# MartinMikkelsen/TensorTrainNumerics.jl

Measured on AMD Instinct MI355X. Metric: TT cores/sec for QTT Laplacian apply+round, d=30 rank-64, higher is better.
Workload: dtype f64

## Files before the change

### include/ttn.h

```cpp
#ifndef TTN_H
#define TTN_H

#include <stdint.h>

#ifdef __cplusplus
extern "C" {
#endif

#define TTN_OK                 0
#define TTN_ERR_DIMS          -1
#define TTN_ERR_BOND_INDEX    -2
#define TTN_ERR_SWEEPS        -3
#define TTN_ERR_CENTER        -4
#define TTN_ERR_CAPACITY      -5
#define TTN_ERR_ARG           -6
#define TTN_ERR_NOT_INIT      -7
#define TTN_ERR_UNSUPPORTED   -8
#define TTN_ERR_NO_CONVERGENCE -9
#define TTN_ERR_SINGULAR      -10

int         ttn_init(int device);
int         ttn_finalize(void);
const char* ttn_version(void);
const char* ttn_last_error_string(void);
// ... 126 lines not shown
int ttn_add(ttn_tt_t x, ttn_tt_t y, ttn_tt_t z);
int ttn_scale(double a, ttn_tt_t x, ttn_tt_t y);
int ttn_scale_batch(const double* a, ttn_tt_t x, ttn_tt_t y);
int ttn_orthogonalize(ttn_tt_t x, int64_t center, ttn_tt_t y);

int ttn_sv_capture(ttn_tt_t h, int enable);
int ttn_sv_get(ttn_tt_t h, int64_t b, int64_t step, double* out, int64_t cap, int64_t* n);

int ttn_timer_begin(void);
int ttn_timer_end(float* ms);
int ttn_event_record(int64_t slot);
int ttn_event_elapsed(int64_t slot_a, int64_t slot_b, float* ms);

int ttn_selftest_gemm(int64_t m, int64_t n, int64_t k, const double* A, const double* B, double* C, double alpha, double beta,
                      int ta, int tb);

int ttn_selftest_lu_solve(int64_t N, const double* K, const double* rhs, double* x_out, int64_t* piv_out, int form);
int ttn_selftest_two_site_apply(int64_t na, int64_t nb, int64_t Rz, const double* G, const double* H, const double* v, double* out);

int ttn_selftest_eig128(const double* G, int64_t n, int64_t r, int64_t nev, double* sig, double* X, int64_t* ticks_rc);
int ttn_selftest_sym_eig(int64_t N, int64_t k, const double* A, double* lam, double* Y);
int ttn_debug_ortho_state(int64_t b, int64_t* out4);

int ttn_apply_f64(int64_t d, const int64_t* dims,
                  const double* const* A_cores, const int64_t* A_rks,
                  const double* const* X_cores, const int64_t* X_rks,
                  double* const* Y_cores);
int ttn_dot_f64(int64_t d, const int64_t* dims,
                const double* const* A_cores, const int64_t* A_rks,
                const double* const* B_cores, const int64_t* B_rks, double* out);
// ... 65 lines not shown
```

### tensortrainnumerics.jl_amd/_lib.py

```python
from __future__ import annotations

import ctypes as C
import os
import subprocess

_HERE = os.path.dirname(os.path.abspath(__file__))
LIB_PATH = os.environ.get("TTN_LIB") or os.path.join(_HERE, "libttn_hip.so")
CSRC = os.path.join(_HERE, "csrc")
INCLUDE = os.path.join(os.path.dirname(_HERE), "include")

TTN_OK = 0
TTN_ERR_DIMS = -1
TTN_ERR_BOND_INDEX = -2
TTN_ERR_SWEEPS = -3
TTN_ERR_CENTER = -4
TTN_ERR_CAPACITY = -5
TTN_ERR_ARG = -6
TTN_ERR_NOT_INIT = -7
TTN_ERR_UNSUPPORTED = -8
TTN_ERR_NO_CONVERGENCE = -9
TTN_ERR_SINGULAR = -10

i64 = C.c_int64
p_i64 = C.POINTER(C.c_int64)
# ... 88 lines not shown
                                   C.c_void_p, C.c_void_p, C.c_void_p]),
    "ttn_cross_eval": (C.c_int, [C.c_int, i64, i64, pp_f64, p_i64, p_i64, C.c_void_p, C.c_void_p, C.c_void_p, C.c_void_p, C.c_double,
                                 C.c_void_p]),
    "ttn_tdvp_contract_f64": (C.c_int, [C.c_int, C.c_int, i64, p_i64, C.c_void_p, C.c_void_p, C.c_void_p, C.c_void_p, C.c_void_p, C.c_void_p, C.c_int]),
    "ttn_selftest_eig128": (C.c_int, [C.c_void_p, i64, i64, i64, C.c_void_p, C.c_void_p, C.c_void_p]),
    "ttn_selftest_sym_eig": (C.c_int, [i64, i64, C.c_void_p, C.c_void_p, C.c_void_p]),
    "ttn_add": (C.c_int, [handle, handle, handle]),
    "ttn_scale": (C.c_int, [C.c_double, handle, handle]),
    "ttn_scale_batch": (C.c_int, [p_f64, handle, handle]),
    "ttn_orthogonalize": (C.c_int, [handle, i64, handle]),
    "ttn_sv_capture": (C.c_int, [handle, C.c_int]),
    "ttn_sv_get": (C.c_int, [handle, i64, i64, p_f64, i64, p_i64]),
    "ttn_timer_begin": (C.c_int, []),
    "ttn_timer_end": (C.c_int, [C.POINTER(C.c_float)]),
    "ttn_selftest_gemm": (C.c_int, [i64, i64, i64, p_f64, p_f64, p_f64, C.c_double, C.c_double, C.c_int, C.c_int]),
    "ttn_selftest_lu_solve": (C.c_int, [i64, p_f64, p_f64, p_f64, p_i64, C.c_int]),
    "ttn_selftest_two_site_apply": (C.c_int, [i64, i64, i64, p_f64, p_f64, p_f64, p_f64]),
    "ttn_event_record": (C.c_int, [i64]),
    "ttn_event_elapsed": (C.c_int, [i64, i64, C.POINTER(C.c_float)]),
    "ttn_apply_f64": (C.c_int, [i64, p_i64, pp_f64, p_i64, pp_f64, p_i64, pp_f64]),
    "ttn_dot_f64": (C.c_int, [i64, p_i64, pp_f64, p_i64, pp_f64, p_i64, p_f64]),
    "ttn_hadamard_f64": (C.c_int, [i64, p_i64, pp_f64, p_i64, pp_f64, p_i64, pp_f64]),
    "ttn_add_f64": (C.c_int, [i64, p_i64, pp_f64, p_i64, pp_f64, p_i64, pp_f64]),
    "ttn_scale_f64": (C.c_int, [i64, p_i64, C.c_double, pp_f64, p_i64, p_i64, pp_f64, p_i64]),
    "ttn_orthogonalize_f64": (C.c_int, [i64, p_i64, pp_f64, p_i64, i64, pp_f64, p_i64, p_i64]),
    "ttn_compress_f64": (C.c_int, [i64, p_i64, pp_f64, p_i64, i64, C.c_double, i64]),
    "ttn_apply_compress_rank_bound": (C.c_int, [i64, p_i64, p_i64, p_i64, i64, i64, p_i64]),
    "ttn_apply_compress_f64": (C.c_int, [i64, p_i64, pp_f64, p_i64, pp_f64, p_i64, pp_f64, p_i64, i64, C.c_double, i64]),
    "ttn_bond_truncate_f64": (C.c_int, [i64, p_i64, pp_f64, p_i64, i64, i64, C.c_double]),
    "ttn_r_and_d_to_rks": (C.c_int, [i64, p_i64, i64, p_i64, i64, p_i64]),
# ... 131 lines not shown
```

### tensortrainnumerics.jl_amd/csrc/ttn_api.hip

```cpp
#include "../../include/ttn.h"
#include "ttn_common.h"
#include "ttn_stream_kernels.h"
#include "ttn_dense_kernels.h"
#include "ttn_swap_kernels.h"
#include "ttn_selftest_kernels.h"
#include "ttn_dot_kernels.h"
#include "ttn_ortho_kernels.h"
#include "ttn_ortho512.h"
#include "ttn_ortho_ramp.h"
#include "ttn_hsvd_kernels.h"
#include "ttn_resite_kernels.h"
#include "ttn_als_kernels.h"
#include "ttn_als_grid.h"
#include "ttn_eigsolve_kernels.h"
#include "ttn_als_eig_kernels.h"
#include "ttn_eig_kernels.h"
#include "ttn_tdvp_kernels.h"
#include "ttn_densefact_kernels.h"
#include "ttn_cross_kernels.h"
#include "ttn_cross_batch_kernels.h"
#include "ttn_opalg_kernels.h"
#include "ttn_cplx_kernels.h"
#include "ttn_grid_kernels.h"
#include "ttn_grad_kernels.h"
// ... 6 lines not shown
#include <cmath>
#include <cstdio>
#include <cstring>
#include <cstdlib>
#include <mutex>
#include <set>
#include <string>
#include <vector>

extern "C" {
int ttn_wg512_init(void);
size_t ttn_wg512_compress_args_bytes(void);
int ttn_wg512_launch_compress(const void* args, size_t nbytes, int grid, hipStream_t stream);
int ttn_wg512_selftest_eig(const double* G, double* Vst, int n, int r, int nev, double* sig, double* Xout, long long* clk, hipStream_t stream);
int ttn_wg512_selftest_gemm(int m, int n, int k, double* A, double* B, double* C, double alpha, double beta, int ta, int tb, hipStream_t stream);
}

namespace {
std::set<struct ttn_tt_s*> g_live;
std::recursive_mutex g_mu;
bool g_init = false;
int g_device = -1;
hipStream_t g_stream = nullptr;
hipEvent_t g_ev0 = nullptr, g_ev1 = nullptr;
hipEvent_t g_launch_ev0 = nullptr, g_launch_ev1 = nullptr;
bool g_have_launch_ms = false;
size_t g_ortho_state_off = 0;
int g_ortho_state_batch = 0;
long long g_dense_plan[3] = {-1, 0, 0};
long long g_gather_plan[4] = {0, 0, 0, 0};
// ... 174 lines not shown
        {(const void*)k_compress, COMPRESS_LDS_BYTES},
        {(const void*)k_selftest_eig128, COMPRESS_LDS_BYTES},
        {(const void*)k_mals_linsolve, COMPRESS_LDS_BYTES},
        {(const void*)k_als_linsolve, COMPRESS_LDS_BYTES},
        {(const void*)k_two_site_eig, COMPRESS_LDS_BYTES},
        {(const void*)k_als_eig, COMPRESS_LDS_BYTES},
        {(const void*)k_increase_ranks, COMPRESS_LDS_BYTES},
        {(const void*)k_ttv_decomp, COMPRESS_LDS_BYTES},
        {(const void*)k_split_sites, COMPRESS_LDS_BYTES},
        {(const void*)k_swap_chain, COMPRESS_LDS_BYTES},
        {(const void*)k_orthogonalize, ORTHO_LDS_BYTES},
        {(const void*)k_ortho512, O5_LDS_BYTES(TTN_MAX_D * 8)},
        {(const void*)k_dot_fused, DOT_LDS_BYTES(DOT_MAX_D)},
        {(const void*)k_grad_chain, DOT_LDS_BYTES(DOT_MAX_D)},
        {(const void*)k_selftest_gemm, sizeof(double) * GEMM_LDS_TOTAL},
        {(const void*)k_tdvp, TDVP_LDS_BYTES},
        {(const void*)k_lu_panel, LU_PANEL_LDS_BYTES},
        {(const void*)k_lu_trail, sizeof(double) * GEMM_LDS_TOTAL},
        {(const void*)k_selftest_lu, COMPRESS_LDS_BYTES},
        {(const void*)k_selftest_two_site_apply, COMPRESS_LDS_BYTES},
        {(const void*)k_cross_maxvol<false>, TTN_XV_LDS_BYTES},
        {(const void*)k_cross_maxvol<true>, TTN_XV_LDS_BYTES},
        {(const void*)k_zcompress, TTN_ZC_LDS_BYTES},
        {(const void*)k_cross_batch_site, TTN_XB_LDS_BYTES},
        {(const void*)k_expect<0>, EXPECT_LDS_BYTES(EXPECT_MAX_D)},
        {(const void*)k_expect<1>, EXPECT_LDS_BYTES(EXPECT_MAX_D)},
        {(const void*)k_expect<2>, EXPECT_LDS_BYTES(EXPECT_MAX_D)},
        {(const void*)k_expect<3>, EXPECT_LDS_BYTES(EXPECT_MAX_D)},
        {(const void*)k_expect<4>, EXPECT_LDS_BYTES(EXPECT_MAX_D)},
        {(const void*)k_expect<5>, EXPECT_LDS_BYTES(EXPECT_MAX_D)},
// ... 2565 lines not shown
    HIPCHK(hipMalloc((void**)&dC, sizeof(double) * m * n));
    HIPCHK(hipMemcpyAsync(dA, A, sizeof(double) * m * k, hipMemcpyHostToDevice, g_stream));
    HIPCHK(hipMemcpyAsync(dB, B, sizeof(double) * k * n, hipMemcpyHostToDevice, g_stream));
    HIPCHK(hipMemcpyAsync(dC, C, sizeof(double) * m * n, hipMemcpyHostToDevice, g_stream));
    if (getenv("TTN_WG512_SELFTEST") && atoi(getenv("TTN_WG512_SELFTEST"))) {
        const int rc512 = ttn_wg512_selftest_gemm((int)m, (int)n, (int)k, dA, dB, dC, alpha, beta, ta, tb, g_stream);
        if (rc512) return hipfail((hipError_t)rc512, "k_selftest_gemm (512-thread build)");
    } else {
    hipLaunchKernelGGL(k_selftest_gemm, dim3(1), dim3(TTN_WG), sizeof(double) * GEMM_LDS_TOTAL, g_stream, (int)m, (int)n, (int)k,
                       dA, dB, dC, alpha, beta, ta, tb);
    HIPCHK(hipGetLastError());
    }
    HIPCHK(hipMemcpyAsync(C, dC, sizeof(double) * m * n, hipMemcpyDeviceToHost, g_stream));
    HIPCHK(hipStreamSynchronize(g_stream));
    hipFree(dA); hipFree(dB); hipFree(dC);
    return TTN_OK;
}

int ttn_selftest_lu_solve(int64_t N, const double* K, const double* rhs, double* x_out, int64_t* piv_out, int form) {
    std::lock_guard<std::recursive_mutex> lk(g_mu);
    if (!K || !rhs || !x_out || !piv_out || N < 1 || (form != 0 && form != 1) || N > (form == 0 ? TTN_DENSE_LOCAL_MAX_ALS : 8192))
        return fail(TTN_ERR_ARG, "ttn_selftest_lu_solve: need 1 <= N <= 2048 (form 0) / 8192 (form 1) and form 0 or 1");
    NEED_INIT();
    { const int rc = g_lu_flag.ensure(sizeof(int)); if (rc) return rc; }
    int* d_flag = g_lu_flag.as<int>();
    double *dK = nullptr, *dR = nullptr;
    int* dP = nullptr;
    HIPCHK(hipMalloc((void**)&dK, sizeof(double) * N * N));
    HIPCHK(hipMalloc((void**)&dR, sizeof(double) * N));
    HIPCHK(hipMalloc((void**)&dP, sizeof(int) * N));
// ... 1311 lines not shown
```

### tensortrainnumerics.jl_amd/csrc/ttn_dense_kernels.h

```cpp
#pragma once
#include "ttn_wg_prims.h"
#include "ttn_wg_gemm.h"
#include "ttn_wg_lq.h"
#include "ttn_wg_jacobi.h"
#include "ttn_wg_chol.h"

struct CompressArgs {
    TTDev tt;
    long long max_bond;
    double truncerr;
    int sweeps;
    int k_single;
    int k_first, k_last;
    double* scratch;
    long long scratch_stride;
    int pmax, qmax;
    double* sv_out;
    int sv_steps;
    int* status;
    int* sweep_stats;
    int fast;
    int fused;
    TTODev op;
    TTDev x;
// ... 131 lines not shown

__device__ __noinline__ double wg_check_diag_tab(const double* sigs, const double* D, int ldd, int r, double s0, double* tab, double* red) {
    sigs = unip(sigs); D = unip(D); ldd = uni32(ldd); r = uni32(r); s0 = unif64(s0); tab = unip(tab); red = unip(red);
    lds_f64* t = (lds_f64*)tab; lds_f64* ref = t + 128;
    const int tid = threadIdx.x, lane = tid & 63, wave = tid >> 6;
    for (int i = tid; i < r; i += TTN_WG) { const double si = sigs[i]; t[i] = 1.0 / sqrt(s0 * si); ref[i] = si * s0; }
    __syncthreads();
    gmem_f64* Dg = (gmem_f64*)D;
    double worst = 0.0;
    for (int j = wave; j < r; j += TTN_NWAVES) {
        const double tj = t[j];
        for (int i = lane; i < r; i += 64) {
            const double dv = Dg[i + ldd * j];
            const double dev = fabs(dv - ((i == j) ? ref[i] : 0.0)) * (t[i] * tj);
            worst = fmax(worst, dev);
        }
    }
    return unif64(wg_max(worst, red));
}

__device__ __noinline__ double wg_diag_test_t3(const double* Ga, const double* Gb, double* T3, double* tab, double* red) {
    Ga = unip(Ga); Gb = unip(Gb); T3 = unip(T3); tab = unip(tab); red = unip(red);
    lds_f64* sd = (lds_f64*)tab; lds_f64* isd = sd + 64;
    const int tid = threadIdx.x, lane = tid & 63, wave = tid >> 6;
    gmem_f64* Gag = (gmem_f64*)Ga; gmem_f64* Gbg = (gmem_f64*)Gb; gmem_wf64* Tg = (gmem_wf64*)T3;
    for (int i = tid; i < 64; i += TTN_WG) { const double d = Gag[i * 129]; const double sq = (d > 0.0) ? sqrt(d) : 0.0; sd[i] = sq; isd[i] = (d > 0.0) ? 1.0 / sq : -1.0; }
    __syncthreads();
    double w = 0.0;
    const double si = sd[lane], ii = isd[lane];
    constexpr int NJ = 64 / TTN_NWAVES;
// ... 700 lines not shown
    int nsw_total = 0;
    bool done = false;

    if (SWAP == 0 && P.fast && rm < p && rm <= TTN_LDS_COLS && rm >= 2) {
        double sa = 0.0, sb = 0.0;
        sa = wg_absmax(ck, (long long)n1 * Dl * rm, S.red);
        sb = wg_absmax(ck1, (long long)n2 * rm * Dr, S.red);
        bool ok = (sa > 0.0) && (sb > 0.0);
        const double sA = wide ? sa : sb, sB = wide ? sb : sa;
        const double s0 = sA * sB;
        const View Gav = mkview(S.Ga, plain(1), plain(128));
        const View Gbv = mkview(S.Gb, plain(1), plain(128));
        const View Ccv = mkview(S.Cc, plain(1), plain(128));
        bool diagA = false;
        if (ok) {
            wg_syrk(rm, p, tview(Ap), Gav, 1.0 / (sA * sA), lds);
            wg_syrk(rm, q, Bp, Gbv, 1.0 / (sB * sB), lds);
            if (rm == 64 && !(P.fast & 4) && !(P.fast & 8)) {
                const double wmax = wg_diag_test_t3(S.Ga, S.Gb, S.T3, S.Ss, S.red);
                diagA = wmax <= FAST_DIAG_TOL;
            }
            if (diagA) {
            } else if (rm <= TTN_LDS_COLS / 2) {
                for (int e = tid; e < rm * 128; e += TTN_WG) if ((e & 127) < rm) { S.ldsX[e] = S.Ga[e]; S.ldsX[TTN_LDS_IMG / 2 + e] = S.Gb[e]; }
                __syncthreads();
                ok = wg_chol2_lds128(rm, S.ldsX, S.Ts, S.iflag, S.scal + 1) == 0;
                for (int e = tid; e < rm * 128; e += TTN_WG) if ((e & 127) < rm) { S.Ga[e] = S.ldsX[e]; S.Gb[e] = S.ldsX[TTN_LDS_IMG / 2 + e]; }
                __syncthreads();
            } else {
                for (int e = tid; e < rm * 128; e += TTN_WG) if ((e & 127) < rm) S.ldsX[e] = S.Ga[e];
                __syncthreads();
                ok = wg_chol_lds128(rm, S.ldsX, S.red, S.iflag, S.scal + 1) == 0;
// ... 44 lines not shown
                    const int row = e % rm, j = e / rm;
                    const double sj = S.sigs[j], xv = S.ldsX[S.perm[j] * 128 + row];
                    const double rs = sqrt(sj);
                    S.T1[j * 128 + row] = xv * (fa / (sj * sj * rs));
                    S.T2[j * 128 + row] = xv * (fb / (sj * rs));
                }
                __syncthreads();
            }
            const View T1v = mkview(S.T1, plain(1), plain(128));
            const View T2v = mkview(S.T2, plain(1), plain(128));
            double* LfT = S.M;
            double* RfT = S.M + (long long)p * rk;
            const View Lft = mkview(LfT, plain(1), plain(p));
            const View Rft = mkview(RfT, plain(q), plain(1));
            if (diagA) {
                wg_gemm_ra(rk, p, rm, tview(T1v), tview(Ap), tview(Lft), 1.0, lds);
                wg_gemm_ra(rk, q, rm, tview(T2v), Bp, Rft, 1.0, lds);
            } else {
            wg_gemm(rm, rk, rm, tview(Ccv), T1v, mkview(S.T3, plain(1), plain(128)), 1.0, 0.0, lds);
            wg_gemm(rm, rk, rm, Gbv, mkview(S.T3, plain(1), plain(128)), T1v, 1.0, 0.0, lds);
            wg_gemm(p, rk, rm, Ap, T1v, Lft, 1.0, 0.0, lds);
            wg_gemm(rm, rk, rm, Gav, T2v, mkview(S.T3, plain(1), plain(128)), 1.0, 0.0, lds);
            wg_gemm(rk, q, rm, tview(mkview(S.T3, plain(1), plain(128))), Bp, Rft, 1.0, 0.0, lds);
            }
            wg_syrk(rk, p, tview(Lft), mkview(S.T1, plain(1), plain(128)), 1.0, lds);
            wg_syrk(rk, q, Rft, mkview(S.T2, plain(1), plain(128)), 1.0, lds);
            const double e1 = wg_check_diag_tab(S.sigs, S.T1, 128, rk, s0, S.Ts, S.red);
            const double e2 = wg_check_diag_tab(S.sigs, S.T2, 128, rk, s0, S.Ts, S.red);
            ok = (e1 <= FAST_CHECK_TOL) && (e2 <= FAST_CHECK_TOL);
            if (ok) {
                if (P.sv_out && step < P.sv_steps) {
                    double* so = P.sv_out + ((long long)b * P.sv_steps + step) * P.pmax;
                    for (int i = tid; i < P.pmax; i += TTN_WG) so[i] = (i < rm) ? S.sigs[i] * s0 : (i < p ? 0.0 : -1.0);
                }
                const View Rfv = mkview(ck1, plain(n2), Idx{n2, 1, (long long)n2 * r});
                const View Lo = wide ? Lfv : tview(Rfv);
                const View Ro = wide ? Rfv : tview(Lfv);
                __syncthreads();
                wg_copy_to_view(Lo, LfT, p, r, 1, p, rk, 1);
                wg_copy_to_view(Ro, RfT, r, q, q, 1, rk, 0);
                if (tid == 0) *io.rank_out = r;
                __syncthreads();
                done = true;
            }
// ... 288 lines not shown
```

### tensortrainnumerics.jl_amd/csrc/ttn_selftest_kernels.h

```cpp
#pragma once
#include "ttn_wg_gemm.h"

__global__ void TTN_KERNEL_BOUNDS k_selftest_gemm(int m, int n, int k, double* A, double* B, double* C, double alpha,
                                                         double beta, int ta, int tb) {
    extern __shared__ double lds[];
    const View Av = (ta & 1) ? mkview(A, plain(1), plain(m)) : mkview(A, plain(k), plain(1));
    const View Bv = tb ? mkview(B, plain(1), plain(k)) : mkview(B, plain(n), plain(1));
    if (ta & 2) wg_syrk(m, k, Av, mkview(C, plain(n), plain(1)), alpha, lds);
    else if (ta & 4) wg_gemm_ra(m, n, k, Av, Bv, mkview(C, plain(n), plain(1)), alpha, lds);
    else wg_gemm(m, n, k, Av, Bv, mkview(C, plain(n), plain(1)), alpha, beta, lds);
}
```

### tensortrainnumerics.jl_amd/csrc/ttn_wg512.hip

```cpp
#include <hip/hip_runtime.h>
#include <stdint.h>
#include <float.h>
#include <string.h>

#define TTN_WG 512
namespace ttn_wg512 {
#include "ttn_common.h"
#include "ttn_dense_kernels.h"
#include "ttn_swap_kernels.h"
#include "ttn_selftest_kernels.h"
#include "ttn_eig_kernels.h"
}

extern "C" {

int ttn_wg512_init(void) {
    hipError_t e;
    if ((e = hipFuncSetAttribute(reinterpret_cast<const void*>(ttn_wg512::k_compress), hipFuncAttributeMaxDynamicSharedMemorySize, (int)COMPRESS_LDS_BYTES)) != hipSuccess) return (int)e;
    if ((e = hipFuncSetAttribute(reinterpret_cast<const void*>(ttn_wg512::k_selftest_eig128), hipFuncAttributeMaxDynamicSharedMemorySize, (int)COMPRESS_LDS_BYTES)) != hipSuccess) return (int)e;
    if ((e = hipFuncSetAttribute(reinterpret_cast<const void*>(ttn_wg512::k_selftest_gemm), hipFuncAttributeMaxDynamicSharedMemorySize, (int)COMPRESS_LDS_BYTES)) != hipSuccess) return (int)e;
    return 0;
}

size_t ttn_wg512_compress_args_bytes(void) { return sizeof(ttn_wg512::CompressArgs); }
size_t ttn_wg512_lds_bytes(void) { return COMPRESS_LDS_BYTES; }

int ttn_wg512_launch_compress(const void* args, size_t nbytes, int grid, hipStream_t stream) {
    if (nbytes != sizeof(ttn_wg512::CompressArgs)) return (int)hipErrorInvalidValue;
    ttn_wg512::CompressArgs P;
    memcpy(&P, args, sizeof(P));
    hipLaunchKernelGGL(ttn_wg512::k_compress, dim3(grid), dim3(TTN_WG), COMPRESS_LDS_BYTES, stream, P);
    return (int)hipGetLastError();
}

int ttn_wg512_selftest_eig(const double* G, double* Vst, int n, int r, int nev, double* sig, double* Xout, long long* clk, hipStream_t stream) {
    hipLaunchKernelGGL(ttn_wg512::k_selftest_eig128, dim3(1), dim3(TTN_WG), COMPRESS_LDS_BYTES, stream, G, Vst, n, r, nev, sig, Xout, clk);
    return (int)hipGetLastError();
}
int ttn_wg512_selftest_gemm(int m, int n, int k, double* A, double* B, double* C, double alpha, double beta, int ta, int tb, hipStream_t stream) {
    hipLaunchKernelGGL(ttn_wg512::k_selftest_gemm, dim3(1), dim3(TTN_WG), COMPRESS_LDS_BYTES, stream, m, n, k, A, B, C, alpha, beta, ta, tb);
    return (int)hipGetLastError();
}

}
```

### tensortrainnumerics.jl_amd/csrc/ttn_wg_gemm.h

```cpp
#pragma once
#include "ttn_wg_prims.h"

#define GEMM_BK 16
#define GEMM_LD 145
#define GEMM_LDS_DOUBLES (TTN_LDS_IMG + 512)


struct GemmDesc {
    int m, n, k, pad;
    View A, B, C;
    double alpha, beta;
    unsigned long long* amax;
};
#if TTN_WG == 512
#define GEMM_TAB_ENTRIES 704
#define GEMM_KSLAB 512
#define GEMM_SMALL_KMAX 256
#else
#define GEMM_TAB_ENTRIES 1536
#define GEMM_KSLAB 768
#define GEMM_SMALL_KMAX 512
#endif
#define GEMM_DESC_DOUBLES (32 + GEMM_TAB_ENTRIES)
#define GEMM_LDS_TOTAL (GEMM_LDS_DOUBLES + GEMM_DESC_DOUBLES)
// ... 347 lines not shown
#pragma unroll
        for (int j = 0; j < D; ++j)
#pragma unroll
            for (int u = 0; u < NT; ++u) {
                acc[u] = __builtin_amdgcn_mfma_f64_16x16x4f64(a[j][u], b[j][u], acc[u], 0, 0, 0);
                a[j][u] = rp[4 * j * LD + ta[u]]; b[j][u] = rp[4 * j * LD + tb[u]];
                __builtin_amdgcn_sched_barrier(0);
            }
    }
#pragma unroll
    for (int j = 0; j < D; ++j)
#pragma unroll
        for (int u = 0; u < NT; ++u) acc[u] = __builtin_amdgcn_mfma_f64_16x16x4f64(a[j][u], b[j][u], acc[u], 0, 0, 0);
}
template <int N> struct syrk_nt { static constexpr int value = N; };
template <int KC16, int JMAX, int MAXT>
__device__ __noinline__ void wg_syrk_impl(const GemmDesc* dsc_, double* lds) {
    const lds_gdesc* dsc = (const lds_gdesc*)dsc_;
    constexpr int KC = 16 * KC16, RG = TTN_WG / 16;
    const int p = uni32(dsc->m), q = uni32(dsc->k);
    const View A = ldsView(&dsc->A), C = ldsView(&dsc->C);
    const double alpha = unif64(dsc->alpha);
    const int tid = threadIdx.x, lane = tid & 63, wave = tid >> 6;
    const int li = lane & 15, lk = lane >> 4;
    constexpr int LD = (JMAX * RG > 64) ? GEMM_LD : 81;
    static_assert(LD >= JMAX * RG + 16 && KC * LD <= GEMM_LDS_DOUBLES, "a chunk fits the region");
    const int pp = (p + 15) & ~15;
    lds_f64* Cs = (lds_f64*)lds;
    lds_i32* rowT = (lds_i32*)(lds + GEMM_LDS_DOUBLES + 32);
    lds_i32* colT = rowT + 128;
    gmem_f64* Ag = (gmem_f64*)A.p;
    for (int i = tid; i < 128; i += TTN_WG) rowT[i] = (i < p) ? (int)ix(A.r, i) : 0;
    for (int i = tid; i < q; i += TTN_WG) colT[i] = (int)ix(A.c, i);
    const int nt = pp >> 4, ntile = nt * (nt + 1) / 2;
    int t_r[MAXT], t_c[MAXT], ta[MAXT], tb[MAXT], nlive = 0;
#pragma unroll
    for (int u = 0; u < MAXT; ++u) {
        const int t = wave + u * TTN_NWAVES;
        int tr = 0, base = 0;
        while (base + tr + 1 <= t) { base += tr + 1; ++tr; }
        t_r[u] = uni32(tr); t_c[u] = uni32(t - base);
        ta[u] = uni32(16 * tr); tb[u] = uni32(16 * (t - base));
        nlive += (t < ntile) ? 1 : 0;
    }
    nlive = uni32(nlive);
    const int fx = tid & 15, sy = tid >> 4;
    gmem_wf64* Cg = (gmem_wf64*)C.p;
    __syncthreads();
    mfma_acc_t res[MAXT];
#pragma unroll
    for (int u = 0; u < MAXT; ++u) res[u] = (mfma_acc_t){0.0, 0.0, 0.0, 0.0};
    auto body = [&](auto ntc) {
        constexpr int NT = decltype(ntc)::value, NA = NT ? NT : 1;
// ... 8 lines not shown
        {                                                                                                               \
            int co_[KC16];                                                                                              \
            _Pragma("unroll") for (int u = 0; u < KC16; ++u) {                                                           \
                const int kk = (K0) + fx + 16 * u;                                                                      \
                co_[u] = colT[kk < q ? kk : 0];                                                                         \
            }                                                                                                           \
            _Pragma("unroll") for (int j = 0; j < JMAX; ++j) {                                                           \
                const int row = sy + RG * j;                                                                            \
                _Pragma("unroll") for (int u = 0; u < KC16; ++u) {                                                       \
                    const int kk = (K0) + fx + 16 * u;                                                                  \
                    v[j][u] = Ag[(row < p && kk < q) ? ro[j] + co_[u] : 0];                                             \
                }                                                                                                       \
            }                                                                                                           \
        }
        SYRK_LOAD(0)
        for (int k0 = 0; k0 < q; k0 += KC) {
#pragma unroll
            for (int j = 0; j < JMAX; ++j) {
                const int row = sy + RG * j;
#pragma unroll
                for (int u = 0; u < KC16; ++u) {
                    const int kl = fx + 16 * u;
                    if (row < pp) Cs[kl * LD + row] = (row < p && k0 + kl < q) ? v[j][u] : 0.0;
                }
            }
            __syncthreads();
            if (k0 + KC < q) { SYRK_LOAD(k0 + KC) }
            const int ksteps = (q - k0 < KC) ? (q - k0 + 3) >> 2 : KC / 4;
            if constexpr (NT > 0) syrk_ksteps<NT, LD, KC / 4>(acc, Cs + lk * LD + li, ksteps, ta, tb);
            __syncthreads();
        }
#undef SYRK_LOAD
#pragma unroll
        for (int u = 0; u < NT; ++u) res[u] = acc[u];
    };
    if (nlive == MAXT) body(syrk_nt<MAXT>{});
    else if (MAXT > 1 && nlive == MAXT - 1) body(syrk_nt<(MAXT > 1 ? MAXT - 1 : 0)>{});
    else if (MAXT > 2 && nlive == MAXT - 2) body(syrk_nt<(MAXT > 2 ? MAXT - 2 : 0)>{});
    else if (MAXT > 3 && nlive == MAXT - 3) body(syrk_nt<(MAXT > 3 ? MAXT - 3 : 0)>{});
    else if (MAXT > 4 && nlive == MAXT - 4) body(syrk_nt<(MAXT > 4 ? MAXT - 4 : 0)>{});
    else body(syrk_nt<0>{});
    static_assert(MAXT <= 5, "one copy of the body per number of live tiles");
#pragma unroll
    for (int u = 0; u < MAXT; ++u) {
        if (u >= nlive) continue;
#pragma unroll
        for (int reg = 0; reg < 4; ++reg) {
            const int gi = 16 * t_r[u] + lk + 4 * reg, gj = 16 * t_c[u] + li;
            if (gi < p && gj < p) {
                const double val = alpha * res[u][reg];
                Cg[ix(C.r, gi) + ix(C.c, gj)] = val;
                if (t_r[u] != t_c[u]) Cg[ix(C.r, gj) + ix(C.c, gi)] = val;
            }
        }
    }
    __syncthreads();
}

__device__ inline void wg_syrk(int p, int q, View A, View G, double alpha, double* lds) {
    if (p > 128 || q > SYRK_QMAX) { wg_gemm(p, p, q, A, tview(A), G, alpha, 0.0, lds); return; }
    GemmDesc* dsc = reinterpret_cast<GemmDesc*>(lds + GEMM_LDS_DOUBLES);
    __syncthreads();
    if (threadIdx.x == 0) { dsc->m = p; dsc->n = p; dsc->k = q; dsc->pad = 0; dsc->A = A; dsc->C = G; dsc->alpha = alpha; dsc->beta = 0.0; dsc->amax = nullptr; }
    __syncthreads();
    TTN_SETPRIO_GEMM();
#if TTN_WG == 512
    if (p > 64) wg_syrk_impl<3, 4, 5>(dsc, lds);
    else wg_syrk_impl<6, 2, 2>(dsc, lds);
#else
    if (p > 64) wg_syrk_impl<6, 2, 3>(dsc, lds);
    else wg_syrk_impl<6, 1, 1>(dsc, lds);
#endif
    TTN_SETPRIO_BASE();
}

#define GEMM_RA_NMAX (2 * GEMM_TAB_ENTRIES - 320)
#define RA_RING 3
template <int NB, int LD>
__device__ __forceinline__ mfma_acc_t ra_ksteps(const double* areg, const lds_f64* bp) {
    mfma_acc_t acc = (mfma_acc_t){0.0, 0.0, 0.0, 0.0};
    double b[RA_RING];
#pragma unroll
    for (int t = 0; t < RA_RING; ++t) b[t] = bp[4 * t * LD];
    __builtin_amdgcn_sched_barrier(0);
#pragma unroll
    for (int ks = 0; ks < 8 * NB; ++ks) {
        acc = __builtin_amdgcn_mfma_f64_16x16x4f64(areg[ks], b[ks % RA_RING], acc, 0, 0, 0);
// ... 82 lines not shown

__device__ inline void wg_gemm_ra(int m, int n, int k, View A, View B, View C, double alpha, double* lds) {
#if TTN_WG != 512
    wg_gemm(m, n, k, A, B, C, alpha, 0.0, lds);
#else
    if (m > 64 || k > 128 || n > GEMM_RA_NMAX || n < 64) { wg_gemm(m, n, k, A, B, C, alpha, 0.0, lds); return; }
    GemmDesc* dsc = reinterpret_cast<GemmDesc*>(lds + GEMM_LDS_DOUBLES);
    __syncthreads();
    if (threadIdx.x == 0) { dsc->m = m; dsc->n = n; dsc->k = k; dsc->pad = 0; dsc->A = A; dsc->B = B; dsc->C = C; dsc->alpha = alpha; dsc->beta = 0.0; dsc->amax = nullptr; }
    __syncthreads();
    TTN_SETPRIO_GEMM();
    wg_gemm_ra_impl(dsc, lds);
    TTN_SETPRIO_BASE();
#endif
}
```

Baseline: 640,400.

## Run paired SYRK and register-A GEMMs concurrently as two workgroup teams

Adds wg_syrk2 and wg_gemm_ra2, which split the workgroup into two half-size teams so that two independent small SYRKs or GEMMs (left and right factors in the compress step) run at the same time instead of back to back. It also fuses the two diagonal checks into a single pass. This aims to cut barrier count and raise MFMA utilisation for rank-64 problems, where one product leaves much of the workgroup idle. In exchange each team has fewer threads and a smaller LDS share, and the code adds new size limits and fallback paths plus selftest entry points.

```diff
diff --git a/include/ttn.h b/include/ttn.h
--- a/include/ttn.h
+++ b/include/ttn.h
@@ -164,6 +164,12 @@
 
 int ttn_selftest_gemm(int64_t m, int64_t n, int64_t k, const double* A, const double* B, double* C, double alpha, double beta,
                       int ta, int tb);
+
+int ttn_selftest_syrk2(int64_t p1, int64_t q1, const double* A1, double* G1, double alpha1, int ta1,
+                       int64_t p2, int64_t q2, const double* A2, double* G2, double alpha2, int ta2, int pair);
+
+int ttn_selftest_gemm_ra2(int64_t m1, int64_t n1, int64_t k1, const double* A1, const double* B1, double* C1, double alpha1, int f1,
+                          int64_t m2, int64_t n2, int64_t k2, const double* A2, const double* B2, double* C2, double alpha2, int f2, int pair);
 
 int ttn_selftest_lu_solve(int64_t N, const double* K, const double* rhs, double* x_out, int64_t* piv_out, int form);
 int ttn_selftest_two_site_apply(int64_t na, int64_t nb, int64_t Rz, const double* G, const double* H, const double* v, double* out);
diff --git a/tensortrainnumerics.jl_amd/_lib.py b/tensortrainnumerics.jl_amd/_lib.py
--- a/tensortrainnumerics.jl_amd/_lib.py
+++ b/tensortrainnumerics.jl_amd/_lib.py
@@ -126,6 +126,8 @@
     "ttn_timer_begin": (C.c_int, []),
     "ttn_timer_end": (C.c_int, [C.POINTER(C.c_float)]),
     "ttn_selftest_gemm": (C.c_int, [i64, i64, i64, p_f64, p_f64, p_f64, C.c_double, C.c_double, C.c_int, C.c_int]),
+    "ttn_selftest_syrk2": (C.c_int, [i64, i64, p_f64, p_f64, C.c_double, C.c_int, i64, i64, p_f64, p_f64, C.c_double, C.c_int, C.c_int]),
+    "ttn_selftest_gemm_ra2": (C.c_int, [i64, i64, i64, p_f64, p_f64, p_f64, C.c_double, C.c_int, i64, i64, i64, p_f64, p_f64, p_f64, C.c_double, C.c_int, C.c_int]),
     "ttn_selftest_lu_solve": (C.c_int, [i64, p_f64, p_f64, p_f64, p_i64, C.c_int]),
     "ttn_selftest_two_site_apply": (C.c_int, [i64, i64, i64, p_f64, p_f64, p_f64, p_f64]),
     "ttn_event_record": (C.c_int, [i64]),
diff --git a/tensortrainnumerics.jl_amd/csrc/ttn_api.hip b/tensortrainnumerics.jl_amd/csrc/ttn_api.hip
--- a/tensortrainnumerics.jl_amd/csrc/ttn_api.hip
+++ b/tensortrainnumerics.jl_amd/csrc/ttn_api.hip
@@ -44,6 +44,10 @@
 int ttn_wg512_launch_compress(const void* args, size_t nbytes, int grid, hipStream_t stream);
 int ttn_wg512_selftest_eig(const double* G, double* Vst, int n, int r, int nev, double* sig, double* Xout, long long* clk, hipStream_t stream);
 int ttn_wg512_selftest_gemm(int m, int n, int k, double* A, double* B, double* C, double alpha, double beta, int ta, int tb, hipStream_t stream);
+int ttn_wg512_selftest_syrk2(int p1, int q1, double* A1, double* G1, double alpha1, int ta1, int p2, int q2, double* A2, double* G2, double alpha2, int ta2,
+                             int pair, hipStream_t stream);
+int ttn_wg512_selftest_gemm_ra2(int m1, int n1, int k1, double* A1, double* B1, double* C1, double alpha1, int f1,
+                                int m2, int n2, int k2, double* A2, double* B2, double* C2, double alpha2, int f2, int pair, hipStream_t stream);
 }
 
 namespace {
@@ -248,6 +252,8 @@
         {(const void*)k_dot_fused, DOT_LDS_BYTES(DOT_MAX_D)},
         {(const void*)k_grad_chain, DOT_LDS_BYTES(DOT_MAX_D)},
         {(const void*)k_selftest_gemm, sizeof(double) * GEMM_LDS_TOTAL},
+        {(const void*)k_selftest_syrk2, sizeof(double) * GEMM_LDS_TOTAL},
+        {(const void*)k_selftest_gemm_ra2, sizeof(double) * GEMM_LDS_TOTAL},
         {(const void*)k_tdvp, TDVP_LDS_BYTES},
         {(const void*)k_lu_panel, LU_PANEL_LDS_BYTES},
         {(const void*)k_lu_trail, sizeof(double) * GEMM_LDS_TOTAL},
@@ -2843,6 +2849,70 @@
     HIPCHK(hipMemcpyAsync(C, dC, sizeof(double) * m * n, hipMemcpyDeviceToHost, g_stream));
     HIPCHK(hipStreamSynchronize(g_stream));
     hipFree(dA); hipFree(dB); hipFree(dC);
+    return TTN_OK;
+}
+
+int ttn_selftest_syrk2(int64_t p1, int64_t q1, const double* A1, double* G1, double alpha1, int ta1,
+                       int64_t p2, int64_t q2, const double* A2, double* G2, double alpha2, int ta2, int pair) {
+    std::lock_guard<std::recursive_mutex> lk(g_mu);
+    NEED_INIT();
+    if (!A1 || !G1 || !A2 || !G2 || p1 < 1 || q1 < 1 || p2 < 1 || q2 < 1 || p1 > 4096 || p2 > 4096 || q1 > 16384 || q2 > 16384)
+        return fail(TTN_ERR_ARG, "bad argument");
+    double *dA1 = nullptr, *dA2 = nullptr, *dG1 = nullptr, *dG2 = nullptr;
+    HIPCHK(hipMalloc((void**)&dA1, sizeof(double) * p1 * q1));
+    HIPCHK(hipMalloc((void**)&dA2, sizeof(double) * p2 * q2));
+    HIPCHK(hipMalloc((void**)&dG1, sizeof(double) * p1 * p1));
+    HIPCHK(hipMalloc((void**)&dG2, sizeof(double) * p2 * p2));
+    HIPCHK(hipMemcpyAsync(dA1, A1, sizeof(double) * p1 * q1, hipMemcpyHostToDevice, g_stream));
+    HIPCHK(hipMemcpyAsync(dA2, A2, sizeof(double) * p2 * q2, hipMemcpyHostToDevice, g_stream));
+    HIPCHK(hipMemcpyAsync(dG1, G1, sizeof(double) * p1 * p1, hipMemcpyHostToDevice, g_stream));
+    HIPCHK(hipMemcpyAsync(dG2, G2, sizeof(double) * p2 * p2, hipMemcpyHostToDevice, g_stream));
+    if (getenv("TTN_WG512_SELFTEST") && atoi(getenv("TTN_WG512_SELFTEST"))) {
+        const int rc512 = ttn_wg512_selftest_syrk2((int)p1, (int)q1, dA1, dG1, alpha1, ta1, (int)p2, (int)q2, dA2, dG2, alpha2, ta2, pair, g_stream);
+        if (rc512) return hipfail((hipError_t)rc512, "k_selftest_syrk2 (512-thread build)");
+    } else {
+        hipLaunchKernelGGL(k_selftest_syrk2, dim3(1), dim3(TTN_WG), sizeof(double) * GEMM_LDS_TOTAL, g_stream, (int)p1, (int)q1, dA1, dG1, alpha1, ta1,
+                           (int)p2, (int)q2, dA2, dG2, alpha2, ta2, pair);
+        HIPCHK(hipGetLastError());
+    }
+    HIPCHK(hipMemcpyAsync(G1, dG1, sizeof(double) * p1 * p1, hipMemcpyDeviceToHost, g_stream));
+    HIPCHK(hipMemcpyAsync(G2, dG2, sizeof(double) * p2 * p2, hipMemcpyDeviceToHost, g_stream));
+    HIPCHK(hipStreamSynchronize(g_stream));
+    hipFree(dA1); hipFree(dA2); hipFree(dG1); hipFree(dG2);
+    return TTN_OK;
+}
+
+int ttn_selftest_gemm_ra2(int64_t m1, int64_t n1, int64_t k1, const double* A1, const double* B1, double* C1, double alpha1, int f1,
+                          int64_t m2, int64_t n2, int64_t k2, const double* A2, const double* B2, double* C2, double alpha2, int f2, int pair) {
+    std::lock_guard<std::recursive_mutex> lk(g_mu);
+    NEED_INIT();
+    const int64_t dm[2] = {m1, m2}, dn[2] = {n1, n2}, dk[2] = {k1, k2};
+    const double* hA[2] = {A1, A2};
+    const double* hB[2] = {B1, B2};
+    double* hC[2] = {C1, C2};
+    for (int i = 0; i < 2; ++i)
+        if (!hA[i] || !hB[i] || !hC[i] || dm[i] < 1 || dn[i] < 1 || dk[i] < 1 || dm[i] > 4096 || dn[i] > 4096 || dk[i] > 4096) return fail(TTN_ERR_ARG, "bad argument");
+    double *dA[2] = {nullptr, nullptr}, *dB[2] = {nullptr, nullptr}, *dC[2] = {nullptr, nullptr};
+    for (int i = 0; i < 2; ++i) {
+        HIPCHK(hipMalloc((void**)&dA[i], sizeof(double) * dm[i] * dk[i]));
+        HIPCHK(hipMalloc((void**)&dB[i], sizeof(double) * dk[i] * dn[i]));
+        HIPCHK(hipMalloc((void**)&dC[i], sizeof(double) * dm[i] * dn[i]));
+        HIPCHK(hipMemcpyAsync(dA[i], hA[i], sizeof(double) * dm[i] * dk[i], hipMemcpyHostToDevice, g_stream));
+        HIPCHK(hipMemcpyAsync(dB[i], hB[i], sizeof(double) * dk[i] * dn[i], hipMemcpyHostToDevice, g_stream));
+        HIPCHK(hipMemcpyAsync(dC[i], hC[i], sizeof(double) * dm[i] * dn[i], hipMemcpyHostToDevice, g_stream));
+    }
+    if (getenv("TTN_WG512_SELFTEST") && atoi(getenv("TTN_WG512_SELFTEST"))) {
+        const int rc512 = ttn_wg512_selftest_gemm_ra2((int)m1, (int)n1, (int)k1, dA[0], dB[0], dC[0], alpha1, f1, (int)m2, (int)n2, (int)k2, dA[1], dB[1], dC[1],
+                                                      alpha2, f2, pair, g_stream);
+        if (rc512) return hipfail((hipError_t)rc512, "k_selftest_gemm_ra2 (512-thread build)");
+    } else {
+        hipLaunchKernelGGL(k_selftest_gemm_ra2, dim3(1), dim3(TTN_WG), sizeof(double) * GEMM_LDS_TOTAL, g_stream, (int)m1, (int)n1, (int)k1, dA[0], dB[0], dC[0],
+                           alpha1, f1, (int)m2, (int)n2, (int)k2, dA[1], dB[1], dC[1], alpha2, f2, pair);
+        HIPCHK(hipGetLastError());
+    }
+    for (int i = 0; i < 2; ++i) HIPCHK(hipMemcpyAsync(hC[i], dC[i], sizeof(double) * dm[i] * dn[i], hipMemcpyDeviceToHost, g_stream));
+    HIPCHK(hipStreamSynchronize(g_stream));
+    for (int i = 0; i < 2; ++i) { hipFree(dA[i]); hipFree(dB[i]); hipFree(dC[i]); }
     return TTN_OK;
 }
 
diff --git a/tensortrainnumerics.jl_amd/csrc/ttn_dense_kernels.h b/tensortrainnumerics.jl_amd/csrc/ttn_dense_kernels.h
--- a/tensortrainnumerics.jl_amd/csrc/ttn_dense_kernels.h
+++ b/tensortrainnumerics.jl_amd/csrc/ttn_dense_kernels.h
@@ -169,6 +169,25 @@
             const double dv = Dg[i + ldd * j];
             const double dev = fabs(dv - ((i == j) ? ref[i] : 0.0)) * (t[i] * tj);
             worst = fmax(worst, dev);
+        }
+    }
+    return unif64(wg_max(worst, red));
+}
+
+__device__ __noinline__ double wg_check_diag_tab2(const double* sigs, const double* D1, const double* D2, int ldd, int r, double s0, double* tab, double* red) {
+    sigs = unip(sigs); D1 = unip(D1); D2 = unip(D2); ldd = uni32(ldd); r = uni32(r); s0 = unif64(s0); tab = unip(tab); red = unip(red);
+    lds_f64* t = (lds_f64*)tab; lds_f64* ref = t + 128;
+    const int tid = threadIdx.x, lane = tid & 63, wave = tid >> 6;
+    for (int i = tid; i < r; i += TTN_WG) { const double si = sigs[i]; t[i] = 1.0 / sqrt(s0 * si); ref[i] = si * s0; }
+    __syncthreads();
+    gmem_f64* D1g = (gmem_f64*)D1; gmem_f64* D2g = (gmem_f64*)D2;
+    double worst = 0.0;
+    for (int j = wave; j < r; j += TTN_NWAVES) {
+        const double tj = t[j];
+        for (int i = lane; i < r; i += 64) {
+            const double d1 = D1g[i + ldd * j], d2 = D2g[i + ldd * j];
+            const double rf = (i == j) ? ref[i] : 0.0, sc = t[i] * tj;
+            worst = fmax(worst, fmax(fabs(d1 - rf) * sc, fabs(d2 - rf) * sc));
         }
     }
     return unif64(wg_max(worst, red));
@@ -899,8 +918,7 @@
         const View Ccv = mkview(S.Cc, plain(1), plain(128));
         bool diagA = false;
         if (ok) {
-            wg_syrk(rm, p, tview(Ap), Gav, 1.0 / (sA * sA), lds);
-            wg_syrk(rm, q, Bp, Gbv, 1.0 / (sB * sB), lds);
+            wg_syrk2(rm, p, tview(Ap), Gav, 1.0 / (sA * sA), rm, q, Bp, Gbv, 1.0 / (sB * sB), lds);
             if (rm == 64 && !(P.fast & 4) && !(P.fast & 8)) {
                 const double wmax = wg_diag_test_t3(S.Ga, S.Gb, S.T3, S.Ss, S.red);
                 diagA = wmax <= FAST_DIAG_TOL;
@@ -975,8 +993,7 @@
             const View Lft = mkview(LfT, plain(1), plain(p));
             const View Rft = mkview(RfT, plain(q), plain(1));
             if (diagA) {
-                wg_gemm_ra(rk, p, rm, tview(T1v), tview(Ap), tview(Lft), 1.0, lds);
-                wg_gemm_ra(rk, q, rm, tview(T2v), Bp, Rft, 1.0, lds);
+                wg_gemm_ra2(rk, p, rm, tview(T1v), tview(Ap), tview(Lft), 1.0, rk, q, rm, tview(T2v), Bp, Rft, 1.0, lds);
             } else {
             wg_gemm(rm, rk, rm, tview(Ccv), T1v, mkview(S.T3, plain(1), plain(128)), 1.0, 0.0, lds);
             wg_gemm(rm, rk, rm, Gbv, mkview(S.T3, plain(1), plain(128)), T1v, 1.0, 0.0, lds);
@@ -984,11 +1001,8 @@
             wg_gemm(rm, rk, rm, Gav, T2v, mkview(S.T3, plain(1), plain(128)), 1.0, 0.0, lds);
             wg_gemm(rk, q, rm, tview(mkview(S.T3, plain(1), plain(128))), Bp, Rft, 1.0, 0.0, lds);
             }
-            wg_syrk(rk, p, tview(Lft), mkview(S.T1, plain(1), plain(128)), 1.0, lds);
-            wg_syrk(rk, q, Rft, mkview(S.T2, plain(1), plain(128)), 1.0, lds);
-            const double e1 = wg_check_diag_tab(S.sigs, S.T1, 128, rk, s0, S.Ts, S.red);
-            const double e2 = wg_check_diag_tab(S.sigs, S.T2, 128, rk, s0, S.Ts, S.red);
-            ok = (e1 <= FAST_CHECK_TOL) && (e2 <= FAST_CHECK_TOL);
+            wg_syrk2(rk, p, tview(Lft), mkview(S.T1, plain(1), plain(128)), 1.0, rk, q, Rft, mkview(S.T2, plain(1), plain(128)), 1.0, lds);
+            ok = wg_check_diag_tab2(S.sigs, S.T1, S.T2, 128, rk, s0, S.Ts, S.red) <= FAST_CHECK_TOL;
             if (ok) {
                 if (P.sv_out && step < P.sv_steps) {
                     double* so = P.sv_out + ((long long)b * P.sv_steps + step) * P.pmax;
diff --git a/tensortrainnumerics.jl_amd/csrc/ttn_selftest_kernels.h b/tensortrainnumerics.jl_amd/csrc/ttn_selftest_kernels.h
--- a/tensortrainnumerics.jl_amd/csrc/ttn_selftest_kernels.h
+++ b/tensortrainnumerics.jl_amd/csrc/ttn_selftest_kernels.h
@@ -10,3 +10,26 @@
     else if (ta & 4) wg_gemm_ra(m, n, k, Av, Bv, mkview(C, plain(n), plain(1)), alpha, lds);
     else wg_gemm(m, n, k, Av, Bv, mkview(C, plain(n), plain(1)), alpha, beta, lds);
 }
+
+__global__ void TTN_KERNEL_BOUNDS k_selftest_syrk2(int p1, int q1, double* A1, double* G1, double alpha1, int ta1,
+                                                   int p2, int q2, double* A2, double* G2, double alpha2, int ta2, int pair) {
+    extern __shared__ double lds[];
+    const View A1v = ta1 ? mkview(A1, plain(1), plain(p1)) : mkview(A1, plain(q1), plain(1));
+    const View A2v = ta2 ? mkview(A2, plain(1), plain(p2)) : mkview(A2, plain(q2), plain(1));
+    const View G1v = mkview(G1, plain(p1), plain(1)), G2v = mkview(G2, plain(p2), plain(1));
+    if (pair) wg_syrk2(p1, q1, A1v, G1v, alpha1, p2, q2, A2v, G2v, alpha2, lds);
+    else { wg_syrk(p1, q1, A1v, G1v, alpha1, lds); wg_syrk(p2, q2, A2v, G2v, alpha2, lds); }
+}
+
+__global__ void TTN_KERNEL_BOUNDS k_selftest_gemm_ra2(int m1, int n1, int k1, double* A1, double* B1, double* C1, double alpha1, int f1,
+                                                      int m2, int n2, int k2, double* A2, double* B2, double* C2, double alpha2, int f2, int pair) {
+    extern __shared__ double lds[];
+    const View A1v = (f1 & 1) ? mkview(A1, plain(1), plain(m1)) : mkview(A1, plain(k1), plain(1));
+    const View B1v = (f1 & 2) ? mkview(B1, plain(1), plain(k1)) : mkview(B1, plain(n1), plain(1));
+    const View C1v = (f1 & 4) ? mkview(C1, plain(1), plain(m1)) : mkview(C1, plain(n1), plain(1));
+    const View A2v = (f2 & 1) ? mkview(A2, plain(1), plain(m2)) : mkview(A2, plain(k2), plain(1));
+    const View B2v = (f2 & 2) ? mkview(B2, plain(1), plain(k2)) : mkview(B2, plain(n2), plain(1));
+    const View C2v = (f2 & 4) ? mkview(C2, plain(1), plain(m2)) : mkview(C2, plain(n2), plain(1));
+    if (pair) wg_gemm_ra2(m1, n1, k1, A1v, B1v, C1v, alpha1, m2, n2, k2, A2v, B2v, C2v, alpha2, lds);
+    else { wg_gemm_ra(m1, n1, k1, A1v, B1v, C1v, alpha1, lds); wg_gemm_ra(m2, n2, k2, A2v, B2v, C2v, alpha2, lds); }
+}
diff --git a/tensortrainnumerics.jl_amd/csrc/ttn_wg512.hip b/tensortrainnumerics.jl_amd/csrc/ttn_wg512.hip
--- a/tensortrainnumerics.jl_amd/csrc/ttn_wg512.hip
+++ b/tensortrainnumerics.jl_amd/csrc/ttn_wg512.hip
@@ -19,6 +19,8 @@
     if ((e = hipFuncSetAttribute(reinterpret_cast<const void*>(ttn_wg512::k_compress), hipFuncAttributeMaxDynamicSharedMemorySize, (int)COMPRESS_LDS_BYTES)) != hipSuccess) return (int)e;
     if ((e = hipFuncSetAttribute(reinterpret_cast<const void*>(ttn_wg512::k_selftest_eig128), hipFuncAttributeMaxDynamicSharedMemorySize, (int)COMPRESS_LDS_BYTES)) != hipSuccess) return (int)e;
     if ((e = hipFuncSetAttribute(reinterpret_cast<const void*>(ttn_wg512::k_selftest_gemm), hipFuncAttributeMaxDynamicSharedMemorySize, (int)COMPRESS_LDS_BYTES)) != hipSuccess) return (int)e;
+    if ((e = hipFuncSetAttribute(reinterpret_cast<const void*>(ttn_wg512::k_selftest_syrk2), hipFuncAttributeMaxDynamicSharedMemorySize, (int)COMPRESS_LDS_BYTES)) != hipSuccess) return (int)e;
+    if ((e = hipFuncSetAttribute(reinterpret_cast<const void*>(ttn_wg512::k_selftest_gemm_ra2), hipFuncAttributeMaxDynamicSharedMemorySize, (int)COMPRESS_LDS_BYTES)) != hipSuccess) return (int)e;
     return 0;
 }
 
@@ -41,5 +43,16 @@
     hipLaunchKernelGGL(ttn_wg512::k_selftest_gemm, dim3(1), dim3(TTN_WG), COMPRESS_LDS_BYTES, stream, m, n, k, A, B, C, alpha, beta, ta, tb);
     return (int)hipGetLastError();
 }
+int ttn_wg512_selftest_syrk2(int p1, int q1, double* A1, double* G1, double alpha1, int ta1, int p2, int q2, double* A2, double* G2, double alpha2, int ta2,
+                             int pair, hipStream_t stream) {
+    hipLaunchKernelGGL(ttn_wg512::k_selftest_syrk2, dim3(1), dim3(TTN_WG), COMPRESS_LDS_BYTES, stream, p1, q1, A1, G1, alpha1, ta1, p2, q2, A2, G2, alpha2, ta2, pair);
+    return (int)hipGetLastError();
+}
+int ttn_wg512_selftest_gemm_ra2(int m1, int n1, int k1, double* A1, double* B1, double* C1, double alpha1, int f1,
+                                int m2, int n2, int k2, double* A2, double* B2, double* C2, double alpha2, int f2, int pair, hipStream_t stream) {
+    hipLaunchKernelGGL(ttn_wg512::k_selftest_gemm_ra2, dim3(1), dim3(TTN_WG), COMPRESS_LDS_BYTES, stream, m1, n1, k1, A1, B1, C1, alpha1, f1,
+                       m2, n2, k2, A2, B2, C2, alpha2, f2, pair);
+    return (int)hipGetLastError();
+}
 
 }
diff --git a/tensortrainnumerics.jl_amd/csrc/ttn_wg_gemm.h b/tensortrainnumerics.jl_amd/csrc/ttn_wg_gemm.h
--- a/tensortrainnumerics.jl_amd/csrc/ttn_wg_gemm.h
+++ b/tensortrainnumerics.jl_amd/csrc/ttn_wg_gemm.h
@@ -385,29 +385,36 @@
         for (int u = 0; u < NT; ++u) acc[u] = __builtin_amdgcn_mfma_f64_16x16x4f64(a[j][u], b[j][u], acc[u], 0, 0, 0);
 }
 template <int N> struct syrk_nt { static constexpr int value = N; };
-template <int KC16, int JMAX, int MAXT>
-__device__ __noinline__ void wg_syrk_impl(const GemmDesc* dsc_, double* lds) {
-    const lds_gdesc* dsc = (const lds_gdesc*)dsc_;
-    constexpr int KC = 16 * KC16, RG = TTN_WG / 16;
+#define SYRK2_TAB (GEMM_TAB_ENTRIES - 32)
+#define SYRK2_QMAX (SYRK2_TAB - 64)
+template <int KC16, int JMAX, int MAXT, int TEAMS>
+__device__ __forceinline__ void syrk_body(const GemmDesc* dsc_, double* lds) {
+    constexpr int TWG = TTN_WG / TEAMS, TNW = TTN_NWAVES / TEAMS, NROW = 128 / TEAMS;
+    const int team = (TEAMS == 1) ? 0 : uni32((int)threadIdx.x / TWG);
+    const lds_gdesc* dsc = (const lds_gdesc*)dsc_ + team;
+    constexpr int KC = 16 * KC16, RG = TWG / 16;
     const int p = uni32(dsc->m), q = uni32(dsc->k);
+    int qall = q;
+    if constexpr (TEAMS == 2) { const int qo = uni32(((const lds_gdesc*)dsc_ + (1 - team))->k); qall = q > qo ? q : qo; }
     const View A = ldsView(&dsc->A), C = ldsView(&dsc->C);
     const double alpha = unif64(dsc->alpha);
-    const int tid = threadIdx.x, lane = tid & 63, wave = tid >> 6;
+    const int tid = threadIdx.x - team * TWG, lane = tid & 63, wave = tid >> 6;
     const int li = lane & 15, lk = lane >> 4;
     constexpr int LD = (JMAX * RG > 64) ? GEMM_LD : 81;
-    static_assert(LD >= JMAX * RG + 16 && KC * LD <= GEMM_LDS_DOUBLES, "a chunk fits the region");
+    static_assert(LD >= JMAX * RG + 16 && TEAMS * KC * LD <= GEMM_LDS_DOUBLES, "a chunk fits the region");
+    static_assert(TEAMS == 1 || (TEAMS == 2 && JMAX * RG == NROW), "two teams: 64 rows each");
     const int pp = (p + 15) & ~15;
-    lds_f64* Cs = (lds_f64*)lds;
-    lds_i32* rowT = (lds_i32*)(lds + GEMM_LDS_DOUBLES + 32);
-    lds_i32* colT = rowT + 128;
+    lds_f64* Cs = (lds_f64*)lds + team * (KC * LD);
+    lds_i32* rowT = (lds_i32*)(lds + GEMM_LDS_DOUBLES + 32 * TEAMS) + team * SYRK2_TAB;
+    lds_i32* colT = rowT + NROW;
     gmem_f64* Ag = (gmem_f64*)A.p;
-    for (int i = tid; i < 128; i += TTN_WG) rowT[i] = (i < p) ? (int)ix(A.r, i) : 0;
-    for (int i = tid; i < q; i += TTN_WG) colT[i] = (int)ix(A.c, i);
+    for (int i = tid; i < NROW; i += TWG) rowT[i] = (i < p) ? (int)ix(A.r, i) : 0;
+    for (int i = tid; i < q; i += TWG) colT[i] = (int)ix(A.c, i);
     const int nt = pp >> 4, ntile = nt * (nt + 1) / 2;
     int t_r[MAXT], t_c[MAXT], ta[MAXT], tb[MAXT], nlive = 0;
 #pragma unroll
     for (int u = 0; u < MAXT; ++u) {
-        const int t = wave + u * TTN_NWAVES;
+        const int t = wave + u * TNW;
         int tr = 0, base = 0;
         while (base + tr + 1 <= t) { base += tr + 1; ++tr; }
         t_r[u] = uni32(tr); t_c[u] = uni32(t - base);
@@ -446,7 +453,7 @@
             }                                                                                                           \
         }
         SYRK_LOAD(0)
-        for (int k0 = 0; k0 < q; k0 += KC) {
+        for (int k0 = 0; k0 < qall; k0 += KC) {
 #pragma unroll
             for (int j = 0; j < JMAX; ++j) {
                 const int row = sy + RG * j;
@@ -459,7 +466,9 @@
             __syncthreads();
             if (k0 + KC < q) { SYRK_LOAD(k0 + KC) }
             const int ksteps = (q - k0 < KC) ? (q - k0 + 3) >> 2 : KC / 4;
-            if constexpr (NT > 0) syrk_ksteps<NT, LD, KC / 4>(acc, Cs + lk * LD + li, ksteps, ta, tb);
+            if constexpr (NT > 0) {
+                if (TEAMS == 1 || ksteps > 0) syrk_ksteps<NT, LD, KC / 4>(acc, Cs + lk * LD + li, ksteps, ta, tb);
+            }
             __syncthreads();
         }
 #undef SYRK_LOAD
@@ -488,6 +497,15 @@
     }
     __syncthreads();
 }
+template <int KC16, int JMAX, int MAXT>
+__device__ __noinline__ void wg_syrk_impl(const GemmDesc* dsc_, double* lds) { syrk_body<KC16, JMAX, MAXT, 1>(dsc_, lds); }
+__device__ __noinline__ void wg_syrk2_impl(const GemmDesc* dsc_, double* lds) {
+#if TTN_WG == 512
+    syrk_body<3, 4, 3, 2>(dsc_, lds);
+#else
+    syrk_body<3, 2, 2, 2>(dsc_, lds);
+#endif
+}
 
 __device__ inline void wg_syrk(int p, int q, View A, View G, double alpha, double* lds) {
     if (p > 128 || q > SYRK_QMAX) { wg_gemm(p, p, q, A, tview(A), G, alpha, 0.0, lds); return; }
@@ -503,6 +521,25 @@
     if (p > 64) wg_syrk_impl<6, 2, 3>(dsc, lds);
     else wg_syrk_impl<6, 1, 1>(dsc, lds);
 #endif
+    TTN_SETPRIO_BASE();
+}
+
+__device__ inline void wg_syrk2(int p1, int q1, View A1, View G1, double alpha1, int p2, int q2, View A2, View G2, double alpha2, double* lds) {
+    if (p1 > 64 || p2 > 64 || q1 > SYRK2_QMAX || q2 > SYRK2_QMAX) {
+        wg_syrk(p1, q1, A1, G1, alpha1, lds);
+        wg_syrk(p2, q2, A2, G2, alpha2, lds);
+        return;
+    }
+    GemmDesc* dsc = reinterpret_cast<GemmDesc*>(lds + GEMM_LDS_DOUBLES);
+    static_assert(2 * sizeof(GemmDesc) <= 64 * sizeof(double), "two descriptors in front of the two-team tables");
+    __syncthreads();
+    if (threadIdx.x == 0) {
+        dsc[0].m = p1; dsc[0].n = p1; dsc[0].k = q1; dsc[0].pad = 0; dsc[0].A = A1; dsc[0].C = G1; dsc[0].alpha = alpha1; dsc[0].beta = 0.0; dsc[0].amax = nullptr;
+        dsc[1].m = p2; dsc[1].n = p2; dsc[1].k = q2; dsc[1].pad = 0; dsc[1].A = A2; dsc[1].C = G2; dsc[1].alpha = alpha2; dsc[1].beta = 0.0; dsc[1].amax = nullptr;
+    }
+    __syncthreads();
+    TTN_SETPRIO_GEMM();
+    wg_syrk2_impl(dsc, lds);
     TTN_SETPRIO_BASE();
 }
 
@@ -615,3 +652,109 @@
     TTN_SETPRIO_BASE();
 #endif
 }
+
+#if TTN_WG == 512
+#define GEMM_RA2_NMAX (SYRK2_TAB - 192)
+__device__ __noinline__ void wg_gemm_ra2_impl(const GemmDesc* dsc_, double* lds) {
+    constexpr int TWG = TTN_WG / 2, NC = 32, LD = 49, KMAX = 64;
+    constexpr int KR = KMAX / (TWG / NC);
+    static_assert(TWG == 256 && 2 * KMAX * LD <= GEMM_LDS_DOUBLES, "one chunk per team holds all of k");
+    const int team = uni32((int)threadIdx.x / TWG);
+    const lds_gdesc* dsc = (const lds_gdesc*)dsc_ + team;
+    const int m = uni32(dsc->m), n = uni32(dsc->n), k = uni32(dsc->k);
+    const int no = uni32(((const lds_gdesc*)dsc_ + (1 - team))->n), nall = n > no ? n : no;
+    const View A = ldsView(&dsc->A), B = ldsView(&dsc->B), C = ldsView(&dsc->C);
+    const double alpha = unif64(dsc->alpha);
+    const int tid = threadIdx.x - team * TWG, lane = tid & 63;
+    const int li = lane & 15, lk = lane >> 4;
+    const int rt = uni32(tid >> 6);
+    lds_f64* Bs = (lds_f64*)lds + team * (KMAX * LD);
+    lds_i32* rowA = (lds_i32*)(lds + GEMM_LDS_DOUBLES + 64) + team * SYRK2_TAB;
+    lds_i32* kA = rowA + 64;
+    lds_i32* kB = kA + KMAX;
+    lds_i32* colB = kB + KMAX;
+    for (int i = tid; i < 64; i += TWG) {
+        rowA[i] = (i < m) ? (int)ix(A.r, i) : 0;
+        kA[i] = (i < k) ? (int)ix(A.c, i) : 0;
+        kB[i] = (i < k) ? (int)ix(B.r, i) : 0;
+    }
+    for (int i = tid; i < n; i += TWG) colB[i] = (int)ix(B.c, i);
+    __syncthreads();
+    gmem_f64* Ag = (gmem_f64*)A.p;
+    gmem_f64* Bg = (gmem_f64*)B.p;
+    gmem_wf64* Cg = (gmem_wf64*)C.p;
+    double areg[KMAX / 4];
+    {
+        const int row = rt * 16 + li, ro = rowA[row];
+#pragma unroll
+        for (int ks = 0; ks < KMAX / 4; ++ks) {
+            const int kk = 4 * ks + lk, ka = kA[kk];
+            areg[ks] = Ag[(row < m && kk < k) ? ro + ka : 0];
+        }
+#pragma unroll
+        for (int ks = 0; ks < KMAX / 4; ++ks) { const int kk = 4 * ks + lk; if (!(row < m && kk < k)) areg[ks] = 0.0; }
+    }
+    const int fx = tid % NC, sy = tid / NC;
+    double v[KR];
+#define RA2_LOAD(C0)         \
+    {                                                                                                                   \
+        const int col = (C0) + fx;                                                                                      \
+        const int co = colB[col < n ? col : 0];                                                                         \
+        int kb_[KR];                                                                                                    \
+        _Pragma("unroll") for (int u = 0; u < KR; ++u) kb_[u] = kB[sy + (TWG / NC) * u];                                \
+        _Pragma("unroll") for (int u = 0; u < KR; ++u) {                                                                 \
+            const int kk = sy + (TWG / NC) * u;                                                                         \
+            v[u] = Bg[(col < n && kk < k) ? co + kb_[u] : 0];                                                           \
+        }                                                                                                               \
+    }
+    RA2_LOAD(0)
+    const bool live = rt * 16 < m;
+    const int nb = uni32((((k + 3) >> 2) + 7) >> 3);
+    for (int c0 = 0; c0 < nall; c0 += NC) {
+#pragma unroll
+        for (int u = 0; u < KR; ++u) {
+            const int kk = sy + (TWG / NC) * u;
+            Bs[kk * LD + fx] = (c0 + fx < n && kk < k) ? v[u] : 0.0;
+        }
+        __syncthreads();
+        if (c0 + NC < n) RA2_LOAD(c0 + NC)
+#pragma unroll
+        for (int cg = 0; cg < 2; ++cg) {
+            if (live && c0 + cg * 16 < n) {
+                const lds_f64* bp = Bs + lk * LD + cg * 16 + li;
+                mfma_acc_t acc;
+                if (nb == 2) acc = ra_ksteps<2, LD>(areg, bp);
+                else acc = ra_ksteps<1, LD>(areg, bp);
+#pragma unroll
+                for (int reg = 0; reg < 4; ++reg) {
+                    const int gi = rt * 16 + lk + 4 * reg, gj = c0 + cg * 16 + li;
+                    if (gi < m && gj < n) Cg[ix(C.r, gi) + ix(C.c, gj)] = alpha * acc[reg];
+                }
+            }
+        }
+        __syncthreads();
+    }
+#undef RA2_LOAD
+}
+#endif
+
+__device__ inline void wg_gemm_ra2(int m1, int n1, int k1, View A1, View B1, View C1, double alpha1,
+                                   int m2, int n2, int k2, View A2, View B2, View C2, double alpha2, double* lds) {
+#if TTN_WG == 512
+    if (m1 <= 64 && m2 <= 64 && k1 <= 64 && k2 <= 64 && n1 >= 64 && n2 >= 64 && n1 <= GEMM_RA2_NMAX && n2 <= GEMM_RA2_NMAX) {
+        GemmDesc* dsc = reinterpret_cast<GemmDesc*>(lds + GEMM_LDS_DOUBLES);
+        __syncthreads();
+        if (threadIdx.x == 0) {
+            dsc[0].m = m1; dsc[0].n = n1; dsc[0].k = k1; dsc[0].pad = 0; dsc[0].A = A1; dsc[0].B = B1; dsc[0].C = C1; dsc[0].alpha = alpha1; dsc[0].beta = 0.0; dsc[0].amax = nullptr;
+            dsc[1].m = m2; dsc[1].n = n2; dsc[1].k = k2; dsc[1].pad = 0; dsc[1].A = A2; dsc[1].B = B2; dsc[1].C = C2; dsc[1].alpha = alpha2; dsc[1].beta = 0.0; dsc[1].amax = nullptr;
+        }
+        __syncthreads();
+        TTN_SETPRIO_GEMM();
+        wg_gemm_ra2_impl(dsc, lds);
+        TTN_SETPRIO_BASE();
+        return;
+    }
+#endif
+    wg_gemm_ra(m1, n1, k1, A1, B1, C1, alpha1, lds);
+    wg_gemm_ra(m2, n2, k2, A2, B2, C2, alpha2, lds);
+}
```

New measurement: 656,100 (median of 6 runs). 2.4% higher.
